# uzh-rpg/rpg_ramnet

Hardware: AMD Instinct MI355X
Metric: depth samples/sec (346x260 cropped to 256x344, 5-bin grids, K=5 grids + 1 frame per sample; training step) (higher is better)
Workload: dtype f32; 1 GPU; EventScape-shaped 346x260 -> 256x344 crop, 5 event bins, K=5, batch 8/GPU, seq-len 8, 1xMI355X-per-rank train, state=convgru, SI loss on [image,events4], Adam, backward-weights co-scheduled on a side stream, decoders on a second stream; global_batch=8, seq_len=8, parallelism=dp1

## Files before the change

### include/ramnet_hip.h

```cpp
#ifndef RAMNET_HIP_H
#define RAMNET_HIP_H
#include <stddef.h>
#include <stdint.h>

#ifdef __cplusplus
extern "C" {
#endif

#define RAMNET_ABI_VERSION 27
#define RAMNET_E_BADARG 10001
#define RAMNET_E_UNSUPPORTED 10002

enum ramnet_in_mode {
    RAMNET_IN_PLAIN = 0,
    RAMNET_IN_CAT = 1,
    RAMNET_IN_CAT_MUL = 2,
    RAMNET_IN_UP2X = 3,
    RAMNET_IN_UP2X_SKIP = 4,
    RAMNET_IN_RELUMASK = 5,
    RAMNET_IN_S2D = 6,
    RAMNET_IN_PARITY4 = 7
};

enum ramnet_algo { RAMNET_ALGO_DIRECT = 0, RAMNET_ALGO_WINOGRAD = 1, RAMNET_ALGO_HEAD = 2, RAMNET_ALGO_WINOGRAD24 = 3, RAMNET_ALGO_WINOGRAD_2X4 = 4,
// ... 100 lines not shown
int ramnet_conv_wino_split_ok(const ramnet_conv_desc *d, int force);
size_t ramnet_packed_weight_elems_wino2x4_split(int Cout, int Cin, int transposed);
int ramnet_pack_weight_wino2x4_split(const float *w_oihw, float *wp, int Cout, int Cin, int transposed, void *stream);
size_t ramnet_conv_splitk_floats(const ramnet_conv_desc *d);
int ramnet_wino2x4_config(int min_wgs);
int ramnet_fold_wino_supported(int Cout, int Cin);
size_t ramnet_packed_weight_elems_fold_wino(int Cout, int Cin);
int ramnet_pack_weight_fold_wino(const float *w_oihw, float *wp, int Cout, int Cin, void *stream);
int ramnet_pack_weight_fold_wino_dgrad(const float *w_oihw, float *wp, int Cout, int Cin, void *stream);
int ramnet_pack_border_weights(const float *w_oihw, float *rows, float *cols, float *rows_t, float *cols_t, int Cout, int Cin, void *stream);
int ramnet_fold_wino_variant(const ramnet_conv_desc *d, int force);
size_t ramnet_packed_weight_elems_fold_wino2x3(int Cout, int Cin);
int ramnet_pack_weight_fold_wino2x3(const float *w_oihw, float *wp, int Cout, int Cin, void *stream);
int ramnet_pack_weight_fold_wino2x3_dgrad(const float *w_oihw, float *wp, int Cout, int Cin, void *stream);
int ramnet_fold_unpack_wgrad(float *w4, float *dU, float *wr, float *wc, float *grad, int Cout, int Cin, int CinWs, void *stream);
size_t ramnet_packed_weight_elems_head(int Cin);
int ramnet_head_supported(int Cin, int Cout);
int ramnet_pack_weight_head(const float *w_oihw, float *wp, int Cout, int Cin, void *stream);
int ramnet_pack_weight(const float *w_oihw, float *wp, int Cout, int Cin, int KH, int KW,
                       int transposed, int gates, void *stream);
int ramnet_unpack_wgrad(const float *ws, float *grad_oihw, int Cout, int Cin, int CinWs, int CoutWs, int n_off,
                        int KH, int KW, void *stream);

int ramnet_unpack_wgrad_wino(const float *ws, float *grad_oihw, int Cout, int Cin, int CinWs, int CoutWs, int n_off,
                             void *stream);
int ramnet_unpack_wgrad_wino2x4(const float *ws, float *grad_oihw, int Cout, int Cin, int CinWs, int CoutWs, int n_off,
                                void *stream);

int ramnet_conv_launch(const ramnet_conv_desc *d, void *stream);
int ramnet_conv_launch_multi(const ramnet_conv_desc *descs, int n, void *stream);
// ... 132 lines not shown
```

### rpg_ramnet_amd/_hip.py

```python
import ctypes as C
import os

_PKG = os.path.dirname(os.path.abspath(__file__))
LIB_PATH = os.environ.get("RAMNET_HIP_LIB") or os.path.join(_PKG, "librpg_ramnet_hip.so")

IN_PLAIN, IN_CAT, IN_CAT_MUL, IN_UP2X, IN_UP2X_SKIP, IN_RELUMASK, IN_S2D, IN_PARITY4 = range(8)
ALGO_DIRECT, ALGO_WINOGRAD, ALGO_HEAD, ALGO_WINOGRAD24, ALGO_WINOGRAD_2X4, ALGO_WINOGRAD_2X4_SPLIT, ALGO_DIRECT_SPLIT = 0, 1, 2, 3, 4, 5, 6
ALGO_WINOGRAD24_2X3 = 7
EPI_LINEAR, EPI_RELU, EPI_SIGMOID, EPI_RES_RELU, EPI_GRU_BLEND, EPI_LSTM, EPI_GRU_BWD, EPI_SIGMOID_HR = range(8)

_fp = C.c_void_p


class ConvDesc(C.Structure):
    _fields_ = [
        ("x0", _fp), ("x1", _fp), ("xm", _fp),
        ("ld0", C.c_int), ("ld1", C.c_int), ("ldm", C.c_int),
        ("C0", C.c_int), ("C1", C.c_int), ("in_mode", C.c_int),
        ("B", C.c_int), ("Hin", C.c_int), ("Win", C.c_int),
        ("ntaps", C.c_int), ("stride", C.c_int),
        ("dy", C.c_int8 * 25), ("dx", C.c_int8 * 25), ("wtap", C.c_uint8 * 25),
        ("w", _fp), ("bias", _fp),
        ("Cout", C.c_int), ("Ho", C.c_int), ("Wo", C.c_int), ("HoF", C.c_int), ("WoF", C.c_int),
        ("osy", C.c_int), ("osx", C.c_int), ("ooy", C.c_int), ("oox", C.c_int),
# ... 71 lines not shown
    "ramnet_pack_weight_wino2x4_split": (C.c_int, [_fp, _fp, C.c_int, C.c_int, C.c_int, _fp]),
    "ramnet_conv_splitk_floats": (C.c_size_t, [C.POINTER(ConvDesc)]),
    "ramnet_packed_weight_elems_head": (C.c_size_t, [C.c_int]),
    "ramnet_head_supported": (C.c_int, [C.c_int, C.c_int]),
    "ramnet_pack_weight_head": (C.c_int, [_fp, _fp, C.c_int, C.c_int, _fp]),
    "ramnet_fold_wino_supported": (C.c_int, [C.c_int, C.c_int]),
    "ramnet_packed_weight_elems_fold_wino": (C.c_size_t, [C.c_int, C.c_int]),
    "ramnet_pack_weight_fold_wino": (C.c_int, [_fp, _fp, C.c_int, C.c_int, _fp]),
    "ramnet_pack_weight_fold_wino_dgrad": (C.c_int, [_fp, _fp, C.c_int, C.c_int, _fp]),
    "ramnet_fold_wino_variant": (C.c_int, [C.POINTER(ConvDesc), C.c_int]),
    "ramnet_packed_weight_elems_fold_wino2x3": (C.c_size_t, [C.c_int, C.c_int]),
    "ramnet_pack_weight_fold_wino2x3": (C.c_int, [_fp, _fp, C.c_int, C.c_int, _fp]),
    "ramnet_pack_weight_fold_wino2x3_dgrad": (C.c_int, [_fp, _fp, C.c_int, C.c_int, _fp]),
    "ramnet_pack_border_weights": (C.c_int, [_fp] * 5 + [C.c_int, C.c_int, _fp]),
    "ramnet_fold_unpack_wgrad": (C.c_int, [_fp] * 5 + [C.c_int, C.c_int, C.c_int, _fp]),
    "ramnet_unpad2_fold": (C.c_int, [_fp, _fp, C.c_int, C.c_int, C.c_int, C.c_int, _fp]),
    "ramnet_up2x_border_col2im": (C.c_int, [_fp, _fp, _fp, C.c_int, C.c_int, C.c_int, C.c_int, _fp]),
    "ramnet_pad2_sum": (C.c_int, [_fp, _fp, _fp, C.c_int, C.c_int, C.c_int, C.c_int, _fp]),
    "ramnet_up2x_border_im2col": (C.c_int, [_fp, _fp, _fp, _fp, C.c_int, C.c_int, C.c_int, C.c_int, _fp]),
    "ramnet_pad2_sum_im2col": (C.c_int, [_fp, _fp, _fp, _fp, _fp, C.c_int, C.c_int, C.c_int, C.c_int, _fp]),
    "ramnet_space_to_depth2": (C.c_int, [_fp, _fp, C.c_int, C.c_int, C.c_int, C.c_int, C.c_int, _fp]),
    "ramnet_frame_gather": (C.c_int, [_fp, _fp, _fp, _fp, C.c_int, C.c_int, C.c_int, C.c_int, _fp]),
    "ramnet_unpack_wgrad": (C.c_int, [_fp, _fp] + [C.c_int] * 7 + [_fp]),
    "ramnet_unpack_wgrad_wino": (C.c_int, [_fp, _fp] + [C.c_int] * 5 + [_fp]),
    "ramnet_unpack_wgrad_wino2x4": (C.c_int, [_fp, _fp] + [C.c_int] * 5 + [_fp]),
    "ramnet_conv_launch": (C.c_int, [C.POINTER(ConvDesc), _fp]),
    "ramnet_conv_launch_multi": (C.c_int, [C.POINTER(ConvDesc), C.c_int, _fp]),
    "ramnet_wgrad_launch": (C.c_int, [C.POINTER(WgradDesc), _fp]),
    "ramnet_pred_sigmoid_fwd": (C.c_int, [_fp, C.c_int, C.c_int, _fp, _fp, _fp, C.c_size_t, _fp]),
    "ramnet_pred_sigmoid_bwd": (C.c_int, [_fp, C.c_int, C.c_int, _fp, _fp, _fp, _fp, C.c_int, _fp, _fp, C.c_size_t, _fp]),
    "ramnet_pred_si_scratch_doubles": (C.c_size_t, [C.c_size_t, C.c_int]),
    "ramnet_pred_sigmoid_si_fwd": (C.c_int, [_fp, C.c_int, C.c_int, _fp, _fp, _fp, C.c_size_t, C.c_int, C.POINTER(C.c_void_p), C.c_float, C.c_float,
                                             _fp, _fp, _fp, _fp]),
    "ramnet_pred_sigmoid_si_bwd": (C.c_int, [_fp, C.c_int, C.c_int, _fp, _fp, _fp, C.c_size_t, C.c_int, C.POINTER(C.c_void_p), _fp, _fp, C.c_float,
                                             C.c_float, _fp, C.c_int, _fp, _fp, _fp, C.c_int, _fp]),
    "ramnet_pred_linear_fwd": (C.c_int, [_fp, C.c_int, C.c_int, _fp, _fp, _fp, C.c_size_t, _fp]),
    "ramnet_pred_linear_bwd": (C.c_int, [_fp, C.c_int, C.c_int, _fp, _fp, _fp, C.c_int, _fp, _fp, C.c_size_t, _fp]),
    "ramnet_pred_sigmoid_dgrad": (C.c_int, [C.c_int, _fp, _fp, _fp, _fp, C.c_int, C.c_size_t, _fp]),
    "ramnet_pred_linear_dgrad": (C.c_int, [C.c_int, _fp, _fp, _fp, C.c_int, C.c_size_t, _fp]),
    "ramnet_pred_sigmoid_si_dgrad": (C.c_int, [_fp, C.c_int, C.c_int, _fp, _fp, _fp, C.c_size_t, C.c_int, C.POINTER(C.c_void_p), _fp, _fp, C.c_float,
                                               C.c_float, _fp, C.c_int, C.c_int, _fp]),
    "ramnet_cat_batch_add": (C.c_int, [_fp, C.c_int, C.c_size_t, C.c_int, C.c_int, _fp, _fp, _fp]),
    "ramnet_cat_batch_add_masked": (C.c_int, [_fp, C.c_int, C.c_size_t, C.c_int, C.c_int, _fp, _fp, _fp, _fp]),
# ... 105 lines not shown
```

### rpg_ramnet_amd/csrc/conv_wgrad.hip

```cpp
#include <stdlib.h>
#include "common.hpp"

namespace ramnet {


struct WgradDerived {
    InSrc src;
    int PH, PW, dymin, dxmin;
    int TH;
    int tiles_x, tiles_y, ntiles;
    int tpm, ntt;
    int toff[25];
    int gsy, gsx, goy, gox, HoG, WoG;
};

template <int MAXT, int NSUB, int CSUB = 1>
__global__ void __launch_bounds__(256, CSUB == 2 ? 2 : 1) conv_wgrad_kernel(const ramnet_wgrad_desc p, const WgradDerived q) {
    constexpr int WBN = 32 * NSUB, GQ = WBN / 4;
    constexpr int WCK = 32 * CSUB;
    constexpr int TSTEP = CSUB == 2 ? 1 : 4 / NSUB;
    extern __shared__ __attribute__((aligned(16))) float smem[];
    float *patch = smem;
    float *gsm = smem + q.PH * q.PW * WCK;
    const int tid = threadIdx.x, lane = tid & 63;
// ... 144 lines not shown
    const ramnet_wgrad_desc &d = *dp;
    RAMNET_CHECK_ARG(d.x0 && d.dout && d.dw);
    RAMNET_CHECK_ARG(d.ntaps >= 1 && d.ntaps <= 25 && (d.stride == 1 || d.stride == 2));
    RAMNET_CHECK_ARG(d.B > 0 && d.Ho > 0 && d.Wo > 0 && d.Cout > 0 && d.Cout % 4 == 0 && d.ldg % 4 == 0);
    RAMNET_CHECK_ARG(d.C0 > 0 && d.C0 % 4 == 0 && d.ld0 % 4 == 0);
    const bool cat = d.in_mode == RAMNET_IN_CAT || d.in_mode == RAMNET_IN_CAT_MUL;
    if (cat) RAMNET_CHECK_ARG(d.x1 && d.C1 > 0 && d.C1 % 4 == 0 && d.ld1 % 4 == 0);
    if (d.in_mode == RAMNET_IN_CAT_MUL || d.in_mode == RAMNET_IN_RELUMASK) RAMNET_CHECK_ARG(d.xm && d.ldm % 4 == 0);
    if (d.in_mode == RAMNET_IN_UP2X_SKIP) RAMNET_CHECK_ARG(d.x1 && d.ld1 % 4 == 0);
    if (d.gmask) RAMNET_CHECK_ARG(d.ldgm % 4 == 0);
    RAMNET_CHECK_ARG(d.ld0 >= d.C0 && d.ldg >= d.Cout && (!d.gmask || d.ldgm >= d.Cout));
    if (cat) RAMNET_CHECK_ARG(d.ld1 >= d.C1);
    if (d.in_mode == RAMNET_IN_CAT_MUL) RAMNET_CHECK_ARG(d.ldm >= d.C1);
    if (d.in_mode == RAMNET_IN_RELUMASK) RAMNET_CHECK_ARG(d.ldm >= d.C0);
    RAMNET_CHECK_ARG(d.nseg >= 0 && (d.nseg == 0 || d.algo == RAMNET_ALGO_WINOGRAD_2X4));
    if (d.algo == RAMNET_ALGO_WINOGRAD24) return launch_wgrad_wino24(d, (hipStream_t)stream);
    const bool gdense = d.gsy == 0 && d.gsx == 0 && d.goy == 0 && d.gox == 0 && d.HoG == 0 && d.WoG == 0;
    if (!gdense) RAMNET_CHECK_ARG(d.gsy >= 1 && d.gsx >= 1 && d.goy >= 0 && d.gox >= 0 && (d.Ho - 1) * d.gsy + d.goy < d.HoG &&
                                  (d.Wo - 1) * d.gsx + d.gox < d.WoG && d.algo == RAMNET_ALGO_DIRECT);
    if (d.algo == RAMNET_ALGO_WINOGRAD) return launch_wgrad_wino(d, (hipStream_t)stream);
    if (d.algo == RAMNET_ALGO_WINOGRAD_2X4) return launch_wgrad_wino6(d, (hipStream_t)stream);
    if (d.algo == RAMNET_ALGO_DIRECT_SPLIT) {
        RAMNET_CHECK_ARG(gdense);
        return launch_wgrad_dsplit(d, (hipStream_t)stream);
    }
    if (d.algo == RAMNET_ALGO_HEAD) {
        RAMNET_CHECK_ARG(gdense);
        return launch_head_wgrad(d, (hipStream_t)stream);
    }
    RAMNET_CHECK_ARG(d.algo == RAMNET_ALGO_DIRECT && d.in_mode != RAMNET_IN_S2D);

// ... 43 lines not shown
```

### rpg_ramnet_amd/csrc/conv_wgrad_wino24.hip

```cpp
#include <stdlib.h>
#include "common.hpp"

namespace ramnet {

constexpr int G24_T = 8;

struct Wgrad24Params {
    const float *x, *g, *gm;
    float *dw, *dbias;
    int ldx, ldg, ldgm, Hp, Wp, H2, W2, Hc, Wc, Cin, Cout, tiles_x, tiles_y, ntiles, nbatch, ncob;
    size_t xbytes, gbytes, gmbytes;
};

template <bool GM, bool WCI>
__global__ void __launch_bounds__(512, 1) conv_wgrad_wino24_kernel(const Wgrad24Params p) {
    constexpr int G24_CI = WCI ? 64 : 32, G24_CO = WCI ? 32 : 64;
    constexpr int G24_V = 25 * G24_T * G24_CI, G24_Z = 25 * G24_T * G24_CO;
    extern __shared__ __attribute__((aligned(16))) float smem[];
    float *V = smem;
    float *Z = smem + 2 * G24_V;
    const int tid = threadIdx.x, lane = tid & 63;
    const int wave = __builtin_amdgcn_readfirstlane(tid >> 6);
    const int l31 = lane & 31, kk = lane >> 5;
    const int pg = wave >> 1, ch = wave & 1;
// ... 179 lines not shown
        }
    }
    if (p.dbias != nullptr && blockIdx.y == 0) {
        __syncthreads();
        float *red = smem;
        if (zrole) red[zt * G24_CO + zc] = bsum;
        __syncthreads();
        if (tid < G24_CO) {
            float t = 0.f;
            for (int g = 0; g < 8; ++g) t += red[g * G24_CO + tid];
            if (n0 + tid < p.Cout) atomicAdd(p.dbias + n0 + tid, t);
        }
    }
}

int launch_wgrad_wino24(const ramnet_wgrad_desc &d, hipStream_t st) {
    const bool wci = d.Cout % 64 != 0;
    const int G24_CI = wci ? 64 : 32, G24_CO = wci ? 32 : 64;
    RAMNET_CHECK_ARG(d.in_mode == RAMNET_IN_PLAIN && d.stride == 1 && d.C0 % G24_CI == 0 && d.Cout % 32 == 0);
    RAMNET_CHECK_ARG(d.Hin == d.Ho + 4 && d.Win == d.Wo + 4 && d.HoG == 2 * d.Ho && d.WoG == 2 * d.Wo && d.Ho >= 2 && d.Wo >= 2);
    Wgrad24Params q;
    q.x = d.x0, q.g = d.dout, q.gm = d.gmask, q.dw = d.dw, q.dbias = d.dbias;
    q.ldx = d.ld0, q.ldg = d.ldg, q.ldgm = d.ldgm, q.Hp = d.Hin, q.Wp = d.Win, q.H2 = d.HoG, q.W2 = d.WoG, q.Hc = d.Ho, q.Wc = d.Wo;
    q.Cin = d.C0, q.Cout = d.Cout;
    q.xbytes = (size_t)d.B * d.Hin * d.Win * d.ld0 * 4, q.gbytes = (size_t)d.B * d.HoG * d.WoG * d.ldg * 4;
    q.gmbytes = d.gmask ? (size_t)d.B * d.HoG * d.WoG * d.ldgm * 4 : 0;
    RAMNET_CHECK_ARG(2 * q.xbytes < WOOB && 2 * q.gbytes < WOOB && 2 * q.gmbytes < WOOB);
    q.tiles_x = cdiv(d.Wo, 2), q.tiles_y = cdiv(d.Ho, 2), q.ntiles = q.tiles_x * q.tiles_y * d.B, q.nbatch = cdiv(q.ntiles, G24_T);
    q.ncob = cdiv(d.Cout, G24_CO);
    const int gy = d.C0 / G24_CI, gz = q.ncob * 4;
    int splits = 256 / (gy * gz);
    if (splits > q.nbatch) splits = q.nbatch;
    if (splits < 1) splits = 1;
    const size_t lds = (size_t)2 * 25 * G24_T * (32 + 64) * sizeof(float);
    const dim3 grid(splits, gy, gz);
    auto go = [&](auto kern) -> int {
        RAMNET_FULL_LDS((kern));
        note_kernel("conv_wgrad_wino24_kernel<%d,%d>", d.gmask ? 1 : 0, (int)wci);
        hipLaunchKernelGGL(kern, grid, dim3(512), lds, st, q);
        return 0;
    };
    const int rc = wci ? (d.gmask ? go(conv_wgrad_wino24_kernel<true, true>) : go(conv_wgrad_wino24_kernel<false, true>))
                       : (d.gmask ? go(conv_wgrad_wino24_kernel<true, false>) : go(conv_wgrad_wino24_kernel<false, false>));
    if (rc) return rc;
    RAMNET_LAUNCH_CHECK();
    return 0;
}

}
```

### rpg_ramnet_amd/csrc/conv_wino24.hip

```cpp
#include <stdlib.h>
#include "common.hpp"
#include "conv_plan.hpp"
#include "conv_epilogue.hpp"

typedef float f32x4 __attribute__((ext_vector_type(4)));

namespace ramnet {

constexpr int W24_PS = 512;
constexpr int W24_V = 25 * W24_PS;
constexpr int W23_V = 30 * W24_PS;

__device__ __forceinline__ float2 ld2f(const float *p) { return *reinterpret_cast<const float2 *>(p); }

__device__ __forceinline__ auto make_rsrc(const void *p, unsigned bytes) {
    const unsigned long long a = (unsigned long long)p;
    const unsigned lo = __builtin_amdgcn_readfirstlane((unsigned)a), hi = __builtin_amdgcn_readfirstlane((unsigned)(a >> 32));
    return __builtin_amdgcn_make_buffer_rsrc((void *)(((unsigned long long)hi << 32) | lo), (short)0, (int)bytes, 0x00020000);
}

#ifdef W24_TRACE
__device__ unsigned long long *g_w24_trace;
#define W24_STAMP(chunk_, slot)                                                                                          \
    do {                                                                                                                 \
// ... 586 lines not shown
        const int ci = (int)(r % Cin);
        r /= Cin;
        const int kb = (int)(r % 5), side = (int)(r / 5);
        const int a0 = side == 0 ? 0 : (slot == 0 ? 4 : 3), na = side == 0 ? (slot == 0 ? 2 : 1) : (slot == 0 ? 1 : 2);
        const float *wk = w + ((size_t)co * Cin + ci) * 25;
        float sr = 0.f, sc = 0.f;
        for (int e = 0; e < na; ++e) sr += wk[(a0 + e) * 5 + kb], sc += wk[kb * 5 + (a0 + e)];
        const size_t K = (size_t)kb * Cin + ci, N = (size_t)slot * Cout + co;
        rows[((size_t)side * 5 * Cin + K) * 2 * Cout + N] = -sr;
        cols[((size_t)side * 5 * Cin + K) * 2 * Cout + N] = -sc;
        rows_t[((size_t)side * 2 * Cout + N) * 5 * Cin + K] = -sr;
        cols_t[((size_t)side * 2 * Cout + N) * 5 * Cin + K] = -sc;
    }
}

__global__ void fold_unpack_wgrad_kernel(float *__restrict__ w4, float *__restrict__ dU, float *__restrict__ wr, float *__restrict__ wc,
                                         float *__restrict__ grad, int Cout, int Cin, int CinWs) {
    const float FA[2][4][5] = {{{.25f, 0, 0, 0, 0}, {.75f, .75f, .25f, 0, 0}, {0, .25f, .75f, .75f, .25f}, {0, 0, 0, .25f, .75f}},
                               {{.75f, .25f, 0, 0, 0}, {.25f, .75f, .75f, .25f, 0}, {0, 0, .25f, .75f, .75f}, {0, 0, 0, 0, .25f}}};
    const float G[5][4] = {{0.5f, 0, 0, 0}, {-0.5f, -0.5f, -0.5f, -0.5f}, {-1.f / 6, 1.f / 6, -1.f / 6, 1.f / 6}, {1.f / 6, 1.f / 3, 2.f / 3, 4.f / 3}, {0, 0, 0, 1.f}};
    const size_t total = (size_t)Cout * Cin;
    for (size_t idx = blockIdx.x * (size_t)blockDim.x + threadIdx.x; idx < total; idx += (size_t)gridDim.x * blockDim.x) {
        const int o = (int)(idx % Cout), i = (int)(idx / Cout);
        float g5[25];
        for (int e = 0; e < 25; ++e) g5[e] = 0.f;
        for (int pq = 0; pq < 4; ++pq) {
            const int pp = pq >> 1, qq = pq & 1;
            float d4[16];
            for (int ts = 0; ts < 16; ++ts) {
                float *cell = w4 + ((size_t)(pq * 16 + ts) * CinWs + i) * Cout + o;
                d4[ts] = *cell;
                *cell = 0.f;
            }
            if (dU != nullptr) {
                for (int ab = 0; ab < 25; ++ab) {
                    float *cell = dU + ((size_t)(pq * 25 + ab) * CinWs + i) * Cout + o;
                    const float u = *cell;
                    *cell = 0.f;
                    const int a = ab / 5, b = ab % 5;
                    for (int t = 0; t < 4; ++t)
                        for (int s = 0; s < 4; ++s) d4[t * 4 + s] += G[a][t] * G[b][s] * u;
                }
            }
            for (int t = 0; t < 4; ++t)
                for (int s = 0; s < 4; ++s) {
                    const float v = d4[t * 4 + s];
                    for (int k = 0; k < 5; ++k) {
                        const float fk = FA[pp][t][k] * v;
                        for (int l = 0; l < 5; ++l) g5[k * 5 + l] += fk * FA[qq][s][l];
                    }
                }
        }
        for (int side = 0; side < 2; ++side)
            for (int slot = 0; slot < 2; ++slot) {
                const int a0 = side == 0 ? 0 : (slot == 0 ? 4 : 3), na = side == 0 ? (slot == 0 ? 2 : 1) : (slot == 0 ? 1 : 2);
                for (int kb = 0; kb < 5; ++kb) {
                    float *rc = wr + (((size_t)side * 5 + kb) * Cin + i) * 2 * Cout + (size_t)slot * Cout + o;
                    float *cc = wc + (((size_t)side * 5 + kb) * Cin + i) * 2 * Cout + (size_t)slot * Cout + o;
// ... 45 lines not shown
    const size_t total = (size_t)120 * Cout * Cin;
    return launch_1d(pack_weight_fold_wino_dgrad_kernel<3>, total, stream, w, wp, Cout, Cin, total);
}

extern "C" int ramnet_fold_wino_variant(const ramnet_conv_desc *d, int force) { return d ? fold_wino_variant(*d, force) : 0; }

extern "C" int ramnet_pack_border_weights(const float *w, float *rows, float *cols, float *rows_t, float *cols_t, int Cout, int Cin, void *stream) {
    RAMNET_CHECK_ARG(w && rows && cols && rows_t && cols_t && Cout > 0 && Cin > 0);
    const size_t total = (size_t)2 * 5 * Cin * 2 * Cout;
    return launch_1d(pack_border_weights_kernel, total, stream, w, rows, cols, rows_t, cols_t, Cout, Cin, total);
}

extern "C" int ramnet_fold_unpack_wgrad(float *w4, float *dU, float *wr, float *wc, float *grad, int Cout, int Cin, int CinWs, void *stream) {
    RAMNET_CHECK_ARG(w4 && wr && wc && grad && Cout > 0 && Cin > 0 && CinWs >= Cin);
    const size_t total = (size_t)Cout * Cin;
    return launch_1d<128>(fold_unpack_wgrad_kernel, total, stream, w4, dU, wr, wc, grad, Cout, Cin, CinWs);
}
```

### rpg_ramnet_amd/ops.py

```python
import contextlib
import ctypes as C
import os as _os

import torch
from torch.autograd import Function

from . import _hip as H

_NULL = None
_ABL_SKIP_WGRAD = _os.environ.get("RAMNET_ABL_SKIP_WGRAD") == "1"
if _ABL_SKIP_WGRAD:
    import warnings as _warnings
    _warnings.warn("RAMNET_ABL_SKIP_WGRAD=1: backward-weights launches are SKIPPED — every weight gradient of this process is zero "
                   "(tuning runs only; unset the variable for anything else)", RuntimeWarning)

_WINOGRAD = True
_WINO_MIN_CIN = 32


def set_winograd(on):
    global _WINOGRAD
    _WINOGRAD = bool(on)


# ... 102 lines not shown
    return Cout % 32 == 0 and Cout >= _FOLD_WINO_MIN_COUT and Cin % (2 * kc) == 0


def set_fold_winograd(on):
    global _FOLD_WINO
    _FOLD_WINO = bool(on)


_FOLD_2X3 = "auto"


def set_fold_winograd_2x3(mode):
    global _FOLD_2X3
    assert mode in ("auto", "off", "force")
    _FOLD_2X3 = mode


def set_fold_upsample(on):
    global _FOLD_UP
    _FOLD_UP = bool(on)


def get_fold_upsample():
    return _FOLD_UP


_RAW_STREAM = getattr(torch._C, "_cuda_getCurrentRawStream", None)
_RAW_DEVICE = getattr(torch._C, "_cuda_getDevice", None)


# ... 213 lines not shown
            nsplit = n
    meta[:] = [kind, nsplit]
    return d


_WDESC_CACHE = {}

_LAYOUTS = {
    "direct": (0, None, "ramnet_unpack_wgrad", H.ALGO_DIRECT),
    "wino": (16, "ramnet_wgrad_wino_slabs", "ramnet_unpack_wgrad_wino", H.ALGO_WINOGRAD),
    "wino6": ("ramnet_wgrad_wino2x4_ws_floats", "ramnet_wgrad_wino2x4_slabs", "ramnet_unpack_wgrad_wino2x4", H.ALGO_WINOGRAD_2X4),
    "dsplit": ("ramnet_wgrad_dsplit_ws_floats", "ramnet_wgrad_dsplit_slabs", "ramnet_unpack_wgrad_dsplit", H.ALGO_DIRECT_SPLIT),
}


def _stamp_layout(dw, kind, slabs, head_cin=0):
    dw.wino, dw.wino6, dw.wg_dsplit = kind == "wino", kind == "wino6", kind == "dsplit"
    dw.slabs, dw.head_cin = slabs, head_cin
    return dw


def _layout_of(dw):
    kind = ("dsplit" if getattr(dw, "wg_dsplit", False) else "wino6" if getattr(dw, "wino6", False) else
            "wino" if getattr(dw, "wino", False) else "direct")
    return kind, getattr(dw, "slabs", 0)


def _wgrad_desc_build(x0, taps, dout, dw, Cout, stride, x1, xm, xm_off, in_mode, C0, C1, Hin, Win, gmask, dbias, Ho, Wo, gview, dw_off, wino24):
    d = H.WgradDesc()
    d.x0, d.x1, d.xm = _p(x0), _p(x1), _p(xm, xm_off)
    d.ld0, d.ld1, d.ldm = ld(x0), (ld(x1) if x1 is not None else 0), (ld(xm) if xm is not None else 0)
    d.C0, d.C1, d.in_mode = (x0.shape[3] if C0 is None else C0), C1, in_mode
    d.B, d.Hin, d.Win = x0.shape[0], (x0.shape[1] if Hin is None else Hin), (x0.shape[2] if Win is None else Win)
    d.ntaps, d.stride = taps.n, stride
    d.dy, d.dx = taps.dy, taps.dx
    d.dout, d.gmask = _p(dout), _p(gmask)
    d.ldg, d.ldgm = ld(dout), (ld(gmask) if gmask is not None else 0)
    d.Cout, d.Ho, d.Wo = Cout, (dout.shape[1] if Ho is None else Ho), (dout.shape[2] if Wo is None else Wo)
    d.dw, d.dbias = _p(dw, dw_off), _p(dbias)
    if gview is not None:
        d.gsy, d.gsx, d.goy, d.gox, d.HoG, d.WoG = gview
    kind, slabs = _layout_of(dw)
    d.algo = _LAYOUTS[kind][3]
    d.dw_slabs = slabs if (kind != "direct" and _WGRAD_SLABS) else 0
    if wino24:
        d.algo = H.ALGO_WINOGRAD24
    hc = getattr(dw, "head_cin", 0)
    if hc and _HEAD and taps.head and stride == 1 and in_mode == H.IN_PLAIN and gview is None and dw_off == 0:
        d.algo, d.head_cin = H.ALGO_HEAD, hc
    if d.algo in (H.ALGO_WINOGRAD, H.ALGO_WINOGRAD_2X4) and C1 and d.C0 % 32:
        raise RuntimeError("Winograd backward-weights needs the concatenation boundary at a multiple of 32 channels")
    return d


def wgrad_launch(x0, taps, dout, dw, Cout, *, stride=1, x1=None, xm=None, xm_off=0, in_mode=H.IN_PLAIN, C0=None,
                 C1=0, Hin=None, Win=None, gmask=None, dbias=None, Ho=None, Wo=None, gview=None, dw_off=0, wino24=False, segs=None, stream=None):
    key = (id(taps), id(dw), _layout_of(dw), getattr(dw, "head_cin", 0), Cout, stride,
           in_mode, C0, C1, Hin, Win, Ho, Wo, gview, dw_off, wino24, xm_off, tuple(x0.shape), x0.stride(2), _sd(x1), _sd(xm), dout.shape[1],
           dout.shape[2], dout.stride(2), _sd(gmask), _WGRAD_SLABS, _HEAD, x0.device.index)
    tmpl = _WDESC_CACHE.get(key) if _DESC_CACHE_ON else None
    if tmpl is not None:
# ... 307 lines not shown
    def __init__(self, weights, biases, gates=1):
        self.weights, self.biases, self.gates = list(weights), list(biases), gates
        w0 = self.weights[0]
        self.Cout = sum(w.shape[0] for w in self.weights)
        self.Cin, self.k = w0.shape[1], w0.shape[2]
        self.CinWs = (self.Cin + 3) // 4 * 4
        self._init_state()

    def _init_state(self):
        self._bias = self._vbias = None
        self._packs = {}
        self._splitk = {}
        self._state_half = self._s2d = None
        self._ws = self._bws = self._slabs = None
        self._ws_fold = None
        self._ws_fold24 = None
        self._fold_used = self._fold24_used = self._ws_used = False
        self._dirty = False
        self._defer = []

    def flush_deferred(self):
        q, self._defer = self._defer, []
        if not q:
            return
        _, _, x0, taps, dout, dw, Cout, kw = q[0]
        if len(q) == 1:
            return wgrad_side(q[0][1], x0, taps, dout, dw, Cout, **kw)
        segs = (H.WgradSeg * len(q))()
        keep = []
        for i, (_, tensors, xi, _, di, _, _, kwi) in enumerate(q):
            segs[i].x0, segs[i].x1, segs[i].xm = _p(xi), _p(kwi.get("x1")), _p(kwi.get("xm"), kwi.get("xm_off", 0))
            segs[i].dout, segs[i].gmask = _p(di), _p(kwi.get("gmask"))
# ... 129 lines not shown
        return self._ws, self._bws

    def grad_ws_fold(self):
        assert len(self.weights) == 1 and self.k == 5
        dev = self.weights[0].device
        if self._bws is None:
            self._bws = torch.zeros(self.Cout, device=dev)
        if self._ws_fold is None:
            self._ws_fold = (torch.zeros(64 * self.CinWs * self.Cout, device=dev),
                             torch.zeros(2, 5 * self.Cin, 2 * self.Cout, device=dev),
                             torch.zeros(2, 5 * self.Cin, 2 * self.Cout, device=dev))
        _Engine.mark(self)
        self._fold_used = True
        return self._ws_fold + (self._bws,)

    def grad_ws_fold24(self):
        if self._ws_fold24 is None:
            self._ws_fold24 = torch.zeros(4 * 25 * self.CinWs * self.Cout, device=self.weights[0].device)
        self._fold24_used = True
        return self._ws_fold24

    def _finalize_fold(self):
        w4, wr, wc = self._ws_fold
        dU = self._ws_fold24 if self._fold24_used else None
        if self.weights[0].requires_grad:
            g = ensure_grad(self.weights[0])
            H.check(H.lib().ramnet_fold_unpack_wgrad(_p(w4), _p(dU), _p(wr), _p(wc), _p(g), self.Cout, self.Cin, self.CinWs, _st()),
                    "ramnet_fold_unpack_wgrad")
        else:
            for t in (w4, dU, wr, wc):
                if t is not None:
                    _zero_later(t)
        self._fold24_used = False
        self._fold_used = False

    def discard(self):
        for t in (self._ws, self._bws, self._ws_fold24) + tuple(self._ws_fold or ()):
            if t is not None:
                t.zero_()
        self._dirty = self._ws_used = self._fold_used = self._fold24_used = False

    def _join_slabs(self):
        kind, ns = _layout_of(self._ws)
        if ns > 1 and kind != "direct":
            H.check(H.lib().ramnet_reduce_slabs(_p(self._ws), ns, self._slab_floats(kind), _st()), "ramnet_reduce_slabs")
            H.check(H.lib().ramnet_reduce_slabs(_p(self._bws), ns, self.Cout, _st()), "ramnet_reduce_slabs")

    def _zero_ws(self):
        kind, ns = _layout_of(self._ws)
        n, ns = self._slab_floats(kind), (1 if kind == "direct" else max(ns, 1))
        joined = ns > 1
        _zero_later(self._ws[:n if joined else min(self._ws.numel(), n * ns)])
        _zero_later(self._bws[:self.Cout if joined else self._bws.numel()])

    def _unpack(self, g, n, off):
# ... 249 lines not shown
    L = H.lib()
    B, Hh, W, Cc = x.shape
    H2, W2 = 2 * Hh, 2 * W
    dev = x.device
    w4, wr, wc, bws = cp.grad_ws_fold()
    with side_work([x, skip, dy, y, xpad], dev):
        a_rows = torch.empty(2, B * W2, 5 * Cc, device=dev)
        a_cols = torch.empty(2, B * H2, 5 * Cc, device=dev)
        if xpad is None:
            xpad = torch.empty(B, Hh + 4, W + 4, Cc, device=dev)
            H.check(L.ramnet_pad2_sum_im2col(_p(x), _p(skip), _p(xpad), _p(a_rows), _p(a_cols), B, Hh, W, Cc, _st()), "ramnet_pad2_sum_im2col")
        else:
            H.check(L.ramnet_up2x_border_im2col(_p(x), _p(skip), _p(a_rows), _p(a_cols), B, Hh, W, Cc, _st()), "ramnet_up2x_border_im2col")
        if _FOLD_WINO_WGRAD and Cc == cp.CinWs and ((Cc % 32 == 0 and cp.Cout % 64 == 0) or
                                                                                 (Cc % 64 == 0 and cp.Cout % 32 == 0)):
            wgrad_launch(xpad, Taps.get("fold", 4, 0, 0, 0), dy, cp.grad_ws_fold24(), cp.Cout, gmask=y, dbias=bws, Ho=Hh, Wo=W,
                         gview=(0, 0, 0, 0, H2, W2), wino24=True)
        else:
            for py in range(2):
                for px in range(2):
                    wgrad_launch(xpad, Taps.get("fold", 4, 0, py, px), dy, w4, cp.Cout, gmask=y, dbias=bws, Ho=Hh, Wo=W,
                                 gview=(2, 2, py, px, H2, W2), dw_off=(py * 2 + px) * 16 * cp.CinWs * cp.Cout)
        g_rows = torch.empty(2, B * W2, 2 * cp.Cout, device=dev)
        g_cols = torch.empty(2, B * H2, 2 * cp.Cout, device=dev)
        H.check(L.ramnet_frame_gather(_p(dy), _p(y), _p(g_rows), _p(g_cols), B, H2, W2, cp.Cout, _st()), "ramnet_frame_gather")
        gemm2(a_rows, g_rows, wr, a_cols, g_cols, wc, trans_a=True, accumulate=True)


_FOLD_DGRAD = True


def set_fold_dgrad(on):
# ... 1098 lines not shown
```

Measured before the change: 245.8 samples/s.

## Add Winograd F(2x2... 2x3) fold-upsample weight-gradient kernel variant with auto selection

```diff
diff --git a/include/ramnet_hip.h b/include/ramnet_hip.h
--- a/include/ramnet_hip.h
+++ b/include/ramnet_hip.h
@@ -138,6 +138,8 @@
 int ramnet_pack_weight_fold_wino2x3(const float *w_oihw, float *wp, int Cout, int Cin, void *stream);
 int ramnet_pack_weight_fold_wino2x3_dgrad(const float *w_oihw, float *wp, int Cout, int Cin, void *stream);
 int ramnet_fold_unpack_wgrad(float *w4, float *dU, float *wr, float *wc, float *grad, int Cout, int Cin, int CinWs, void *stream);
+int ramnet_fold_wgrad_variant(const ramnet_wgrad_desc *d, int force);
+int ramnet_fold_unpack_wgrad2x3(float *w4, float *dU, float *dU3, float *wr, float *wc, float *grad, int Cout, int Cin, int CinWs, void *stream);
 size_t ramnet_packed_weight_elems_head(int Cin);
 int ramnet_head_supported(int Cin, int Cout);
 int ramnet_pack_weight_head(const float *w_oihw, float *wp, int Cout, int Cin, void *stream);
diff --git a/rpg_ramnet_amd/_hip.py b/rpg_ramnet_amd/_hip.py
--- a/rpg_ramnet_amd/_hip.py
+++ b/rpg_ramnet_amd/_hip.py
@@ -109,6 +109,7 @@
     "ramnet_pack_weight_fold_wino2x3_dgrad": (C.c_int, [_fp, _fp, C.c_int, C.c_int, _fp]),
     "ramnet_pack_border_weights": (C.c_int, [_fp] * 5 + [C.c_int, C.c_int, _fp]),
     "ramnet_fold_unpack_wgrad": (C.c_int, [_fp] * 5 + [C.c_int, C.c_int, C.c_int, _fp]),
+    "ramnet_fold_unpack_wgrad2x3": (C.c_int, [_fp] * 6 + [C.c_int, C.c_int, C.c_int, _fp]),
     "ramnet_unpad2_fold": (C.c_int, [_fp, _fp, C.c_int, C.c_int, C.c_int, C.c_int, _fp]),
     "ramnet_up2x_border_col2im": (C.c_int, [_fp, _fp, _fp, C.c_int, C.c_int, C.c_int, C.c_int, _fp]),
     "ramnet_pad2_sum": (C.c_int, [_fp, _fp, _fp, C.c_int, C.c_int, C.c_int, C.c_int, _fp]),
@@ -122,6 +123,7 @@
     "ramnet_conv_launch": (C.c_int, [C.POINTER(ConvDesc), _fp]),
     "ramnet_conv_launch_multi": (C.c_int, [C.POINTER(ConvDesc), C.c_int, _fp]),
     "ramnet_wgrad_launch": (C.c_int, [C.POINTER(WgradDesc), _fp]),
+    "ramnet_fold_wgrad_variant": (C.c_int, [C.POINTER(WgradDesc), C.c_int]),
     "ramnet_pred_sigmoid_fwd": (C.c_int, [_fp, C.c_int, C.c_int, _fp, _fp, _fp, C.c_size_t, _fp]),
     "ramnet_pred_sigmoid_bwd": (C.c_int, [_fp, C.c_int, C.c_int, _fp, _fp, _fp, _fp, C.c_int, _fp, _fp, C.c_size_t, _fp]),
     "ramnet_pred_si_scratch_doubles": (C.c_size_t, [C.c_size_t, C.c_int]),
diff --git a/rpg_ramnet_amd/csrc/conv_wgrad.hip b/rpg_ramnet_amd/csrc/conv_wgrad.hip
--- a/rpg_ramnet_amd/csrc/conv_wgrad.hip
+++ b/rpg_ramnet_amd/csrc/conv_wgrad.hip
@@ -182,7 +182,7 @@
     if (d.in_mode == RAMNET_IN_CAT_MUL) RAMNET_CHECK_ARG(d.ldm >= d.C1);
     if (d.in_mode == RAMNET_IN_RELUMASK) RAMNET_CHECK_ARG(d.ldm >= d.C0);
     RAMNET_CHECK_ARG(d.nseg >= 0 && (d.nseg == 0 || d.algo == RAMNET_ALGO_WINOGRAD_2X4));
-    if (d.algo == RAMNET_ALGO_WINOGRAD24) return launch_wgrad_wino24(d, (hipStream_t)stream);
+    if (d.algo == RAMNET_ALGO_WINOGRAD24 || d.algo == RAMNET_ALGO_WINOGRAD24_2X3) return launch_wgrad_wino24(d, (hipStream_t)stream);
     const bool gdense = d.gsy == 0 && d.gsx == 0 && d.goy == 0 && d.gox == 0 && d.HoG == 0 && d.WoG == 0;
     if (!gdense) RAMNET_CHECK_ARG(d.gsy >= 1 && d.gsx >= 1 && d.goy >= 0 && d.gox >= 0 && (d.Ho - 1) * d.gsy + d.goy < d.HoG &&
                                   (d.Wo - 1) * d.gsx + d.gox < d.WoG && d.algo == RAMNET_ALGO_DIRECT);
diff --git a/rpg_ramnet_amd/csrc/conv_wgrad_wino24.hip b/rpg_ramnet_amd/csrc/conv_wgrad_wino24.hip
--- a/rpg_ramnet_amd/csrc/conv_wgrad_wino24.hip
+++ b/rpg_ramnet_amd/csrc/conv_wgrad_wino24.hip
@@ -217,7 +217,238 @@
     }
 }
 
+constexpr int G23_T = 6, G23_NP = 30;
+
+template <bool GM, bool WCI>
+__global__ void __launch_bounds__(512, 1) conv_wgrad_wino24_kernel_2x3(const Wgrad24Params p) {
+    constexpr int CI = WCI ? 64 : 32, CO = WCI ? 32 : 64;
+    constexpr int NV = G23_NP * G23_T * CI, NZ = G23_NP * G23_T * CO;
+    extern __shared__ __attribute__((aligned(16))) float smem[];
+    float *V = smem;
+    float *Z = smem + 2 * NV;
+    const int tid = threadIdx.x, lane = tid & 63;
+    const int wave = __builtin_amdgcn_readfirstlane(tid >> 6);
+    const int l31 = lane & 31, kk = lane >> 5;
+    const int pg = wave >> 1, ch = wave & 1;
+    const int p0 = pg < 2 ? 8 * pg : 2 + 7 * pg;
+    const int cls = blockIdx.z / p.ncob, cob = blockIdx.z % p.ncob;
+    const int py = cls >> 1, px = cls & 1;
+    const int c0 = blockIdx.y * CI, n0 = cob * CO;
+    const bool vrole = WCI ? wave < 6 : wave >= 5, zrole = WCI ? wave >= 6 : wave < 5;
+    const bool z2 = wave == (WCI ? 6 : 4);
+    const int vi = WCI ? tid : max(tid - 320, 0), zi = WCI ? (wave == 7 ? 128 + lane : lane) : tid;
+    const int vt = vi / CI, vc = vi % CI;
+    const int zt = zi / CO, zc = zi % CO;
+
+    f32x16 acc[8];
+#pragma unroll
+    for (int i = 0; i < 8; ++i)
+#pragma unroll
+        for (int r = 0; r < 16; ++r) acc[i][r] = 0.f;
+
+    float vraw[30], zraw[12], zmraw[GM ? 12 : 1];
+    float bsum = 0.f;
+    bool zcnt = false;
+    struct Walk { int tx, ty, b, T; };
+    const int dT = G23_T * (int)gridDim.x;
+    const int d_tx = dT % p.tiles_x, d_ty = (dT / p.tiles_x) % p.tiles_y, d_b = (dT / p.tiles_x) / p.tiles_y;
+    auto walk_init = [&](Walk &w, int batch, int tile) {
+        w.T = batch * G23_T + tile;
+        int t = w.T;
+        w.tx = t % p.tiles_x;
+        t /= p.tiles_x;
+        w.ty = t % p.tiles_y, w.b = t / p.tiles_y;
+    };
+    auto walk_step = [&](Walk &w, int adv) {
+        w.T += adv * dT;
+        w.tx += adv * d_tx;
+        const int cx = w.tx >= p.tiles_x ? 1 : 0;
+        w.tx -= cx * p.tiles_x;
+        w.ty += adv * d_ty + cx;
+        const int cy = w.ty >= p.tiles_y ? 1 : 0;
+        w.ty -= cy * p.tiles_y;
+        w.b += adv * d_b + cy;
+    };
+    Walk wv, wz, wz2;
+    int lbv = 0, lbz = 0;
+    const auto rx = wino_rsrc(p.x, (unsigned)min((size_t)p.xbytes, (size_t)WOOB));
+    const auto rg = wino_rsrc(p.g, (unsigned)min((size_t)p.gbytes, (size_t)WOOB));
+    const auto rgm = GM ? wino_rsrc(p.gm, (unsigned)min((size_t)p.gmbytes, (size_t)WOOB)) : rg;
+    const bool vch_ok = c0 + vc < p.Cin, zch_ok = n0 + zc < p.Cout;
+    const unsigned zch = (unsigned)(n0 + zc);
+    const int rowB = p.Wp * p.ldx * 4, colB = p.ldx * 4;
+    auto load_v = [&](int batch) {
+        walk_step(wv, batch != lbv ? 1 : 0);
+        lbv = batch;
+        const int wx = 3 * wv.tx + px;
+        const unsigned base = (unsigned)(((wv.b * p.Hp + 2 * wv.ty + py) * p.Wp + wx) * p.ldx + c0 + vc) * 4u;
+        const bool ok = (wv.T < p.ntiles) & vch_ok;
+        const unsigned lane_off = ok ? base : WOOB;
+        const unsigned lane_off4 = (ok & (wx + 4 < p.Wp)) ? base : WOOB;
+#pragma unroll
+        for (int r = 0; r < 5; ++r)
+#pragma unroll
+            for (int c = 0; c < 6; ++c)
+                vraw[r * 6 + c] = __builtin_bit_cast(float, __builtin_amdgcn_raw_buffer_load_b32(rx, (int)((c == 4 ? lane_off4 : lane_off) + (unsigned)(r * rowB)), c * colB, 0));
+    };
+    auto load_z1 = [&](Walk &wz, int o, int adv) {
+        walk_step(wz, adv);
+        const bool tok = (wz.T < p.ntiles) & zch_ok;
+#pragma unroll
+        for (int a = 0; a < 2; ++a)
+#pragma unroll
+            for (int c = 0; c < 3; ++c) {
+                const int oy = 2 * wz.ty + a, ox = 3 * wz.tx + c;
+                const bool ok = tok & (oy < p.Hc) & (ox < p.Wc);
+                const unsigned pix = (unsigned)((wz.b * p.H2 + 2 * oy + py) * p.W2 + 2 * ox + px);
+                const unsigned oob = ok ? 0u : 0x80000000u;
+                zraw[o + a * 3 + c] = __builtin_bit_cast(float, __builtin_amdgcn_raw_buffer_load_b32(rg, (int)(((pix * p.ldg + zch) * 4u) | oob), 0, 0));
+                if (GM) zmraw[o + a * 3 + c] = __builtin_bit_cast(float, __builtin_amdgcn_raw_buffer_load_b32(rgm, (int)(((pix * p.ldgm + zch) * 4u) | oob), 0, 0));
+            }
+    };
+    auto load_z = [&](int batch, bool count) {
+        const int adv = batch != lbz ? 1 : 0;
+        lbz = batch;
+        load_z1(wz, 0, adv);
+        if (z2) load_z1(wz2, 6, adv);
+        zcnt = count;
+    };
+    auto z_mask = [&]() {
+#pragma unroll
+        for (int i = 0; i < 12; ++i) {
+            if (i < 6 || z2) {
+                if (GM) zraw[i] = zmraw[i] > 0.f ? zraw[i] : 0.f;
+                bsum += zcnt ? zraw[i] : 0.f;
+            }
+        }
+    };
+    auto v_cols = [&]() {
+#pragma unroll
+        for (int c = 0; c < 6; ++c) {
+            const float d0 = vraw[c], d1 = vraw[6 + c], d2 = vraw[12 + c], d3 = vraw[18 + c], d4 = vraw[24 + c];
+            vraw[c] = 2.f * (d0 - d2) - d1 + d3;
+            vraw[6 + c] = d3 - d2 - 2.f * d1;
+            vraw[12 + c] = 2.f * d1 - 3.f * d2 + d3;
+            vraw[18 + c] = d3 - d1;
+            vraw[24 + c] = 2.f * (d1 - d3) - d2 + d4;
+        }
+    };
+    auto v_row = [&](float *vbuf, int i) {
+        const float d0 = vraw[i * 6], d1 = vraw[i * 6 + 1], d2 = vraw[i * 6 + 2], d3 = vraw[i * 6 + 3], d4 = vraw[i * 6 + 4], d5 = vraw[i * 6 + 5];
+        float *dst = vbuf + ((i * 6) * G23_T + vt) * CI + vc;
+        const float e = d4 - 0.25f * d2, o = d3 - 0.25f * d1;
+        const float f = d4 - d2, h = 0.5f * (d3 - d1);
+        dst[0 * G23_T * CI] = 0.25f * d0 - 1.25f * d2 + d4;
+        dst[1 * G23_T * CI] = e + o;
+        dst[2 * G23_T * CI] = e - o;
+        dst[3 * G23_T * CI] = f + h;
+        dst[4 * G23_T * CI] = f - h;
+        dst[5 * G23_T * CI] = 0.25f * d1 - 1.25f * d3 + d5;
+    };
+    auto z_row1 = [&](float *zbuf, int i, const float *zraw, int zt) {
+        float w0, w1, w2;
+        if (i == 0) w0 = zraw[0], w1 = zraw[1], w2 = zraw[2];
+        if (i == 1) w0 = zraw[0] + zraw[3], w1 = zraw[1] + zraw[4], w2 = zraw[2] + zraw[5];
+        if (i == 2) w0 = zraw[0] - zraw[3], w1 = zraw[1] - zraw[4], w2 = zraw[2] - zraw[5];
+        if (i == 3) w0 = zraw[0] + 2.f * zraw[3], w1 = zraw[1] + 2.f * zraw[4], w2 = zraw[2] + 2.f * zraw[5];
+        if (i == 4) w0 = zraw[3], w1 = zraw[4], w2 = zraw[5];
+        float *dst = zbuf + ((i * 6) * G23_T + zt) * CO + zc;
+        const float s = w0 + w2, q = w0 + 0.25f * w2;
+        dst[0 * G23_T * CO] = w0;
+        dst[1 * G23_T * CO] = s + w1;
+        dst[2 * G23_T * CO] = s - w1;
+        dst[3 * G23_T * CO] = q + 0.5f * w1;
+        dst[4 * G23_T * CO] = q - 0.5f * w1;
+        dst[5 * G23_T * CO] = w2;
+    };
+    auto z_row = [&](float *zbuf, int i) {
+        z_row1(zbuf, i, zraw, zt);
+        if (z2) z_row1(zbuf, i, zraw + 6, zt + 64 / CO);
+    };
+
+    const int step = gridDim.x;
+    int batch = blockIdx.x;
+    if (batch < p.nbatch) {
+        const int last = batch + ((p.nbatch - 1 - batch) / step) * step;
+        walk_init(wv, batch, vt), walk_init(wz, batch, zt), walk_init(wz2, batch, zt + 64 / CO);
+        lbv = lbz = batch;
+        if (zrole) load_z(batch, true);
+        if (vrole) load_v(batch);
+        if (zrole) {
+            z_mask();
+#pragma unroll
+            for (int i = 0; i < 5; ++i) z_row(Z, i);
+        }
+        if (vrole) {
+            v_cols();
+#pragma unroll
+            for (int i = 0; i < 5; ++i) v_row(V, i);
+        }
+        {
+            const bool more = batch + step <= last;
+            if (zrole) load_z(min(batch + step, last), more);
+            if (vrole) load_v(min(batch + step, last));
+        }
+        __syncthreads();
+        const int aoff = (kk * 3) * CI + (WCI ? ch * 32 : 0) + l31, boff = (kk * 3) * CO + (WCI ? 0 : ch * 32) + l31;
+        int buf = 0;
+        for (; batch <= last; batch += step, buf ^= 1) {
+            const float *vb = V + buf * NV, *zb = Z + buf * NZ;
+            float *vn = V + (buf ^ 1) * NV, *zn = Z + (buf ^ 1) * NZ;
+            const int b2 = min(batch + 2 * step, last);
+            const bool more2 = batch + 2 * step <= last;
+#pragma unroll
+            for (int q = 0; q < 8; ++q) {
+                if (q < 7 || pg < 2) {
+                    const int pos = p0 + q;
+                    const float *ap = vb + pos * (G23_T * CI) + aoff, *bp = zb + pos * (G23_T * CO) + boff;
+                    const float a0 = ap[0], a1 = ap[CI], a2 = ap[2 * CI];
+                    const float b0 = bp[0], b1 = bp[CO], b2v = bp[2 * CO];
+                    __builtin_amdgcn_sched_barrier(0);
+                    acc[q] = __builtin_amdgcn_mfma_f32_32x32x2f32(a0, b0, acc[q], 0, 0, 0);
+                    acc[q] = __builtin_amdgcn_mfma_f32_32x32x2f32(a1, b1, acc[q], 0, 0, 0);
+                    __builtin_amdgcn_sched_barrier(0);
+                    if (q == 0 && zrole) z_mask(), z_row(zn, 0), z_row(zn, 1), z_row(zn, 2);
+                    if (q == 1 && zrole) z_row(zn, 3), z_row(zn, 4), load_z(b2, more2);
+                    if (q == 2 && vrole) v_cols();
+                    if (q == 3 && vrole) v_row(vn, 0), v_row(vn, 1), v_row(vn, 2);
+                    if (q == 4 && vrole) v_row(vn, 3), v_row(vn, 4), load_v(b2);
+                    __builtin_amdgcn_sched_barrier(0);
+                    acc[q] = __builtin_amdgcn_mfma_f32_32x32x2f32(a2, b2v, acc[q], 0, 0, 0);
+                    __builtin_amdgcn_sched_barrier(0);
+                }
+            }
+            __syncthreads();
+        }
+    }
+
+    const int n = n0 + (WCI ? 0 : ch * 32) + l31;
+#pragma unroll
+    for (int q = 0; q < 8; ++q) {
+        if (q < 7 || pg < 2) {
+#pragma unroll
+            for (int r = 0; r < 16; ++r) {
+                const int c = c0 + (WCI ? ch * 32 : 0) + (r & 3) + 8 * (r >> 2) + 4 * kk;
+                if (c < p.Cin && n < p.Cout) atomicAdd(p.dw + (((size_t)cls * G23_NP + p0 + q) * p.Cin + c) * p.Cout + n, acc[q][r]);
+            }
+        }
+    }
+    if (p.dbias != nullptr && blockIdx.y == 0) {
+        __syncthreads();
+        float *red = smem;
+        if (zrole) red[zt * CO + zc] = bsum;
+        if (z2) red[(zt + 64 / CO) * CO + zc] = 0.f;
+        __syncthreads();
+        if (tid < CO) {
+            float t = 0.f;
+            for (int g = 0; g < G23_T; ++g) t += red[g * CO + tid];
+            if (n0 + tid < p.Cout) atomicAdd(p.dbias + n0 + tid, t);
+        }
+    }
+}
+
 int launch_wgrad_wino24(const ramnet_wgrad_desc &d, hipStream_t st) {
+    const bool f23 = d.algo == RAMNET_ALGO_WINOGRAD24_2X3;
     const bool wci = d.Cout % 64 != 0;
     const int G24_CI = wci ? 64 : 32, G24_CO = wci ? 32 : 64;
     RAMNET_CHECK_ARG(d.in_mode == RAMNET_IN_PLAIN && d.stride == 1 && d.C0 % G24_CI == 0 && d.Cout % 32 == 0);
@@ -229,25 +460,41 @@
     q.xbytes = (size_t)d.B * d.Hin * d.Win * d.ld0 * 4, q.gbytes = (size_t)d.B * d.HoG * d.WoG * d.ldg * 4;
     q.gmbytes = d.gmask ? (size_t)d.B * d.HoG * d.WoG * d.ldgm * 4 : 0;
     RAMNET_CHECK_ARG(2 * q.xbytes < WOOB && 2 * q.gbytes < WOOB && 2 * q.gmbytes < WOOB);
-    q.tiles_x = cdiv(d.Wo, 2), q.tiles_y = cdiv(d.Ho, 2), q.ntiles = q.tiles_x * q.tiles_y * d.B, q.nbatch = cdiv(q.ntiles, G24_T);
+    const int tiles_per_batch = f23 ? G23_T : G24_T;
+    q.tiles_x = cdiv(d.Wo, f23 ? 3 : 2), q.tiles_y = cdiv(d.Ho, 2), q.ntiles = q.tiles_x * q.tiles_y * d.B, q.nbatch = cdiv(q.ntiles, tiles_per_batch);
     q.ncob = cdiv(d.Cout, G24_CO);
     const int gy = d.C0 / G24_CI, gz = q.ncob * 4;
     int splits = 256 / (gy * gz);
     if (splits > q.nbatch) splits = q.nbatch;
     if (splits < 1) splits = 1;
-    const size_t lds = (size_t)2 * 25 * G24_T * (32 + 64) * sizeof(float);
+    const size_t lds = (size_t)2 * (f23 ? G23_NP : 25) * tiles_per_batch * (32 + 64) * sizeof(float);
     const dim3 grid(splits, gy, gz);
     auto go = [&](auto kern) -> int {
         RAMNET_FULL_LDS((kern));
-        note_kernel("conv_wgrad_wino24_kernel<%d,%d>", d.gmask ? 1 : 0, (int)wci);
+        note_kernel(f23 ? "conv_wgrad_wino24_kernel_2x3<%d,%d>" : "conv_wgrad_wino24_kernel<%d,%d>", d.gmask ? 1 : 0, (int)wci);
         hipLaunchKernelGGL(kern, grid, dim3(512), lds, st, q);
         return 0;
     };
-    const int rc = wci ? (d.gmask ? go(conv_wgrad_wino24_kernel<true, true>) : go(conv_wgrad_wino24_kernel<false, true>))
+    const int rc = f23 ? (wci ? (d.gmask ? go(conv_wgrad_wino24_kernel_2x3<true, true>) : go(conv_wgrad_wino24_kernel_2x3<false, true>))
+                              : (d.gmask ? go(conv_wgrad_wino24_kernel_2x3<true, false>) : go(conv_wgrad_wino24_kernel_2x3<false, false>)))
+                 : wci ? (d.gmask ? go(conv_wgrad_wino24_kernel<true, true>) : go(conv_wgrad_wino24_kernel<false, true>))
                        : (d.gmask ? go(conv_wgrad_wino24_kernel<true, false>) : go(conv_wgrad_wino24_kernel<false, false>));
     if (rc) return rc;
     RAMNET_LAUNCH_CHECK();
     return 0;
 }
 
+int wgrad_wino24_variant(const ramnet_wgrad_desc &d, int force) {
+    if (d.algo != RAMNET_ALGO_WINOGRAD24 || d.in_mode != RAMNET_IN_PLAIN || d.stride != 1 || d.Ho < 2 || d.Wo < 2 || d.B < 1) return 0;
+    const bool wci = d.Cout % 64 != 0;
+    const int ci = wci ? 64 : 32, co = wci ? 32 : 64;
+    if (d.C0 % ci != 0 || d.Cout % 32 != 0) return 0;
+    if (force) return 1;
+    const long nbatch = ((long)cdiv(d.Wo, 3) * cdiv(d.Ho, 2) * d.B + G23_T - 1) / G23_T;
+    const int per_split = 256 / ((d.C0 / ci) * cdiv(d.Cout, co) * 4);
+    return nbatch >= 24L * (per_split < 1 ? 1 : per_split) ? 1 : 0;
 }
+
+}
+
+extern "C" int ramnet_fold_wgrad_variant(const ramnet_wgrad_desc *d, int force) { return d ? ramnet::wgrad_wino24_variant(*d, force) : 0; }
diff --git a/rpg_ramnet_amd/csrc/conv_wino24.hip b/rpg_ramnet_amd/csrc/conv_wino24.hip
--- a/rpg_ramnet_amd/csrc/conv_wino24.hip
+++ b/rpg_ramnet_amd/csrc/conv_wino24.hip
@@ -624,8 +624,8 @@
     }
 }
 
-__global__ void fold_unpack_wgrad_kernel(float *__restrict__ w4, float *__restrict__ dU, float *__restrict__ wr, float *__restrict__ wc,
-                                         float *__restrict__ grad, int Cout, int Cin, int CinWs) {
+__global__ void fold_unpack_wgrad_kernel(float *__restrict__ w4, float *__restrict__ dU, float *__restrict__ dU3, float *__restrict__ wr,
+                                         float *__restrict__ wc, float *__restrict__ grad, int Cout, int Cin, int CinWs) {
     const float FA[2][4][5] = {{{.25f, 0, 0, 0, 0}, {.75f, .75f, .25f, 0, 0}, {0, .25f, .75f, .75f, .25f}, {0, 0, 0, .25f, .75f}},
                                {{.75f, .25f, 0, 0, 0}, {.25f, .75f, .75f, .25f, 0}, {0, 0, .25f, .75f, .75f}, {0, 0, 0, 0, .25f}}};
     const float G[5][4] = {{0.5f, 0, 0, 0}, {-0.5f, -0.5f, -0.5f, -0.5f}, {-1.f / 6, 1.f / 6, -1.f / 6, 1.f / 6}, {1.f / 6, 1.f / 3, 2.f / 3, 4.f / 3}, {0, 0, 0, 1.f}};
@@ -652,6 +652,16 @@
                         for (int s = 0; s < 4; ++s) d4[t * 4 + s] += G[a][t] * G[b][s] * u;
                 }
             }
+            if (dU3 != nullptr) {
+                for (int ab = 0; ab < 30; ++ab) {
+                    float *cell = dU3 + ((size_t)(pq * 30 + ab) * CinWs + i) * Cout + o;
+                    const float u = *cell;
+                    *cell = 0.f;
+                    const int a = ab / 6, b = ab % 6;
+                    for (int t = 0; t < 4; ++t)
+                        for (int s = 0; s < 4; ++s) d4[t * 4 + s] += G[a][t] * (float)fold_wino_gc(3, b, s) * u;
+                }
+            }
             for (int t = 0; t < 4; ++t)
                 for (int s = 0; s < 4; ++s) {
                     const float v = d4[t * 4 + s];
@@ -727,5 +737,12 @@
 extern "C" int ramnet_fold_unpack_wgrad(float *w4, float *dU, float *wr, float *wc, float *grad, int Cout, int Cin, int CinWs, void *stream) {
     RAMNET_CHECK_ARG(w4 && wr && wc && grad && Cout > 0 && Cin > 0 && CinWs >= Cin);
     const size_t total = (size_t)Cout * Cin;
-    return launch_1d<128>(fold_unpack_wgrad_kernel, total, stream, w4, dU, wr, wc, grad, Cout, Cin, CinWs);
-}
+    return launch_1d<128>(fold_unpack_wgrad_kernel, total, stream, w4, dU, (float *)nullptr, wr, wc, grad, Cout, Cin, CinWs);
+}
+
+extern "C" int ramnet_fold_unpack_wgrad2x3(float *w4, float *dU, float *dU3, float *wr, float *wc, float *grad, int Cout, int Cin, int CinWs,
+                                           void *stream) {
+    RAMNET_CHECK_ARG(w4 && wr && wc && grad && Cout > 0 && Cin > 0 && CinWs >= Cin);
+    const size_t total = (size_t)Cout * Cin;
+    return launch_1d<128>(fold_unpack_wgrad_kernel, total, stream, w4, dU, dU3, wr, wc, grad, Cout, Cin, CinWs);
+}
diff --git a/rpg_ramnet_amd/ops.py b/rpg_ramnet_amd/ops.py
--- a/rpg_ramnet_amd/ops.py
+++ b/rpg_ramnet_amd/ops.py
@@ -140,6 +140,31 @@
     global _FOLD_2X3
     assert mode in ("auto", "off", "force")
     _FOLD_2X3 = mode
+
+
+_FOLD_WGRAD_2X3 = "auto"
+_FOLD_WGRAD_VARIANT = {}
+
+
+def set_fold_winograd_wgrad_2x3(mode):
+    global _FOLD_WGRAD_2X3
+    assert mode in ("auto", "off", "force")
+    _FOLD_WGRAD_2X3 = mode
+
+
+def _fold_wgrad_2x3(B, Hh, W, Cin, Cout):
+    if _FOLD_WGRAD_2X3 == "off":
+        return False
+    key = (B, Hh, W, Cin, Cout, _FOLD_WGRAD_2X3, _DESC_EPOCH)
+    hit = _FOLD_WGRAD_VARIANT.get(key)
+    if hit is None:
+        d = H.WgradDesc()
+        d.algo, d.in_mode, d.stride = H.ALGO_WINOGRAD24, H.IN_PLAIN, 1
+        d.B, d.Hin, d.Win, d.Ho, d.Wo, d.HoG, d.WoG = B, Hh + 4, W + 4, Hh, W, 2 * Hh, 2 * W
+        d.C0 = d.ld0 = Cin
+        d.Cout = d.ldg = d.ldgm = Cout
+        hit = _FOLD_WGRAD_VARIANT[key] = bool(H.lib().ramnet_fold_wgrad_variant(C.byref(d), int(_FOLD_WGRAD_2X3 == "force")))
+    return hit
 
 
 def set_fold_upsample(on):
@@ -383,6 +408,12 @@
 }
 
 
+_FOLD_LAYOUTS = {
+    "fold24": (25, True),
+    "fold23": (30, "2x3"),
+}
+
+
 def _stamp_layout(dw, kind, slabs, head_cin=0):
     dw.wino, dw.wino6, dw.wg_dsplit = kind == "wino", kind == "wino6", kind == "dsplit"
     dw.slabs, dw.head_cin = slabs, head_cin
@@ -413,7 +444,7 @@
     d.algo = _LAYOUTS[kind][3]
     d.dw_slabs = slabs if (kind != "direct" and _WGRAD_SLABS) else 0
     if wino24:
-        d.algo = H.ALGO_WINOGRAD24
+        d.algo = H.ALGO_WINOGRAD24_2X3 if wino24 == "2x3" else H.ALGO_WINOGRAD24
     hc = getattr(dw, "head_cin", 0)
     if hc and _HEAD and taps.head and stride == 1 and in_mode == H.IN_PLAIN and gview is None and dw_off == 0:
         d.algo, d.head_cin = H.ALGO_HEAD, hc
@@ -751,8 +782,8 @@
         self._state_half = self._s2d = None
         self._ws = self._bws = self._slabs = None
         self._ws_fold = None
-        self._ws_fold24 = None
-        self._fold_used = self._fold24_used = self._ws_used = False
+        self._ws_fold24 = self._ws_fold23 = None
+        self._fold_used = self._fold24_used = self._fold23_used = self._ws_used = False
         self._dirty = False
         self._defer = []
 
@@ -912,31 +943,41 @@
         self._fold_used = True
         return self._ws_fold + (self._bws,)
 
-    def grad_ws_fold24(self):
-        if self._ws_fold24 is None:
-            self._ws_fold24 = torch.zeros(4 * 25 * self.CinWs * self.Cout, device=self.weights[0].device)
-        self._fold24_used = True
-        return self._ws_fold24
+    def grad_ws_fold24(self, kind="fold24"):
+        f23 = kind == "fold23"
+        ws = self._ws_fold23 if f23 else self._ws_fold24
+        if ws is None:
+            ws = torch.zeros(4 * _FOLD_LAYOUTS[kind][0] * self.CinWs * self.Cout, device=self.weights[0].device)
+        if f23:
+            self._ws_fold23, self._fold23_used = ws, True
+        else:
+            self._ws_fold24, self._fold24_used = ws, True
+        return ws
 
     def _finalize_fold(self):
         w4, wr, wc = self._ws_fold
         dU = self._ws_fold24 if self._fold24_used else None
+        dU3 = self._ws_fold23 if self._fold23_used else None
         if self.weights[0].requires_grad:
             g = ensure_grad(self.weights[0])
-            H.check(H.lib().ramnet_fold_unpack_wgrad(_p(w4), _p(dU), _p(wr), _p(wc), _p(g), self.Cout, self.Cin, self.CinWs, _st()),
-                    "ramnet_fold_unpack_wgrad")
+            if dU3 is not None:
+                H.check(H.lib().ramnet_fold_unpack_wgrad2x3(_p(w4), _p(dU), _p(dU3), _p(wr), _p(wc), _p(g), self.Cout, self.Cin, self.CinWs, _st()),
+                        "ramnet_fold_unpack_wgrad2x3")
+            else:
+                H.check(H.lib().ramnet_fold_unpack_wgrad(_p(w4), _p(dU), _p(wr), _p(wc), _p(g), self.Cout, self.Cin, self.CinWs, _st()),
+                        "ramnet_fold_unpack_wgrad")
         else:
-            for t in (w4, dU, wr, wc):
+            for t in (w4, dU, dU3, wr, wc):
                 if t is not None:
                     _zero_later(t)
-        self._fold24_used = False
+        self._fold24_used = self._fold23_used = False
         self._fold_used = False
 
     def discard(self):
-        for t in (self._ws, self._bws, self._ws_fold24) + tuple(self._ws_fold or ()):
+        for t in (self._ws, self._bws, self._ws_fold24, self._ws_fold23) + tuple(self._ws_fold or ()):
             if t is not None:
                 t.zero_()
-        self._dirty = self._ws_used = self._fold_used = self._fold24_used = False
+        self._dirty = self._ws_used = self._fold_used = self._fold24_used = self._fold23_used = False
 
     def _join_slabs(self):
         kind, ns = _layout_of(self._ws)
@@ -1216,8 +1257,9 @@
             H.check(L.ramnet_up2x_border_im2col(_p(x), _p(skip), _p(a_rows), _p(a_cols), B, Hh, W, Cc, _st()), "ramnet_up2x_border_im2col")
         if _FOLD_WINO_WGRAD and Cc == cp.CinWs and ((Cc % 32 == 0 and cp.Cout % 64 == 0) or
                                                                                  (Cc % 64 == 0 and cp.Cout % 32 == 0)):
-            wgrad_launch(xpad, Taps.get("fold", 4, 0, 0, 0), dy, cp.grad_ws_fold24(), cp.Cout, gmask=y, dbias=bws, Ho=Hh, Wo=W,
-                         gview=(0, 0, 0, 0, H2, W2), wino24=True)
+            kind = "fold23" if _fold_wgrad_2x3(B, Hh, W, Cc, cp.Cout) else "fold24"
+            wgrad_launch(xpad, Taps.get("fold", 4, 0, 0, 0), dy, cp.grad_ws_fold24(kind), cp.Cout, gmask=y, dbias=bws, Ho=Hh, Wo=W,
+                         gview=(0, 0, 0, 0, H2, W2), wino24=_FOLD_LAYOUTS[kind][1])
         else:
             for py in range(2):
                 for px in range(2):
```

Result: faster. 248.9 samples/s (median of 6 runs) (+1.3%).
